# NCAR/SPERR

Hardware: AMD Instinct MI355X
Metric: compress+decompress GB/s/GPU on 256^3 fp32 chunks @ BPP=2.0; bitstream-exact vs ref (higher is better)
Workload: dtype f64; 1 GPU; synthetic 1024^3 fp32 turbulence per GPU, 256^3 chunks, BPP=2.0, step = compress + decompress, volume and container resident in HBM; chunks_per_gpu=64, parallelism=chunks farmed over 1 GPU(s), no collective

## Files before the change

sperr_amd/csrc/engine.hip:

```cpp
#include <algorithm>
#include <array>
#include <chrono>
#include <cstdlib>
#include <cstring>
#include <atomic>
#include <deque>
#include <map>
#include <memory>
#include <condition_variable>
#include <mutex>
#include <numeric>
#include <thread>
#include <string>
#include <vector>

#include "../../include/sperr_hip.h"
#include "engine_internal.h"
#include "host_container.hpp"
#include "speck_dec.h"
#include "dequant.h"
#include "speck_enc.h"
#include "speck_tree_host.hpp"
#include "outlier.h"
#include "quality.h"
// ... 2438 lines not shown
  d.tileStride = round_up(d.nPixTiles, 32);
  TAKE(d.tileLip, uint32_t, d.tileStride * B);
  TAKE(d.tileRef, uint32_t, d.tileStride * B);
  TAKE(d.tileLipOff, uint32_t, d.tileStride * B);
  TAKE(d.tileRefOff, uint32_t, d.tileStride * B);
  {
    uint8_t* tb = nullptr;
    TAKE(tb, uint8_t, d.tileStride * B);
    d.tileBorn = use_tables(P) ? tb : nullptr;
  }
  d.lipResStride = Npad / 64 + 2;
  TAKE(d.lipSig, uint64_t, d.lipResStride * B);
  TAKE(d.lipNeg, uint64_t, d.lipResStride * B);
  d.tokStride = (2 * N + 1 + 63) / 64 + 2;
  TAKE(d.tokMask, uint64_t, d.tokStride * B);
  TAKE(d.tokCnt, uint32_t, d.tokStride * B);
  TAKE(d.tokOff, uint32_t, d.tokStride * B);
  d.tokSegStride = round_up(d.tokStride / 2048 + 2, 32);
  TAKE(d.tokSegSum, uint32_t, d.tokSegStride * B);
  TAKE(d.tokSegBase, uint32_t, d.tokSegStride * B);
  d.streamStride = (size_t)(maxPayloadBytes / 8) + 4;
  TAKE(d.stream, uint64_t, d.streamStride * B);
  d.levelClass = P.d_levelClass;
  d.levelSlot = P.d_levelSlot;
  d.slotLevel = P.d_slotLevel;
  d.nSlots = P.nSlots;
  d.maskWords = (uint32_t)d.streamStride;
  d.maskStride = (size_t)P.nSlots * d.maskWords;
  TAKE(d.mask, uint64_t, std::max<size_t>(d.maskStride, 1) * B);
  d.prefWords = (d.maskWords + 3u) / 4u;
  d.prefStride = (size_t)P.nSlots * d.prefWords;
  TAKE(d.maskPrefix, uint32_t, std::max<size_t>(d.prefStride, 1) * B);
  d.bornStride = P.ht.nsets + 8;
  d.hiGroupsMax = 8;
  d.bornSeg = (uint32_t)((P.ht.nsets + 8) / 16 + 64);
  d.bornPitch = d.bornStride + (size_t)d.bornSeg * d.hiGroupsMax;
  TAKE(d.bornPacked, uint64_t, d.bornPitch * B);
  TAKE(d.bornPosLev, uint64_t, d.bornPitch * B);
  d.lisStamps = nullptr;
  if (g_lis_stamps_on) {
    TAKE(d.lisStamps, uint64_t, 64 * B);
  }
  d.queueCap = 28672 + 64;
  static const int hiKcap = tune_getenv("SPERR_HIP_HI_KCAP") ? std::max(2, atoi(tune_getenv("SPERR_HIP_HI_KCAP"))) : 5;
  d.hiK = (uint32_t)std::min(std::max(2, P.maxK), hiKcap);
  static const uint32_t ahead = tune_getenv("SPERR_HIP_HI_AHEAD") ? (uint32_t)atoi(tune_getenv("SPERR_HIP_HI_AHEAD")) : 512u;
  d.hiAhead = ahead;
  static const uint32_t extra = tune_getenv("SPERR_HIP_HI_EXTRA") ? (uint32_t)atoi(tune_getenv("SPERR_HIP_HI_EXTRA")) : 1u;
  d.hiExtra = extra;
  d.hiHop2 = 0;
  d.hiCand = 1;
  d.hiSmemBytes = 148 * 1024;
  d.hiW = hi_window((int)d.hiK, d.hiSmemBytes, d.hiHop2);
  d.queueStride = (size_t)d.queueCap * 4 * d.hiGroupsMax;
  TAKE(d.queue, uint64_t, d.queueStride * B);
  d.hiAhead = std::min(d.hiAhead / 64 * 64, d.hiW / 2);
  d.hiFlagStride = ((d.streamStride * 64 + N) / std::max<uint32_t>(512u, d.hiW - d.hiAhead) + 12) * 4;
  d.mxSlot = P.d_mxSlot;
  d.mxLevelGroup = P.d_mxLevelGroup;
  d.mxS = kMxS;
  d.mxM = kMxM;
  d.mxQ = kMxQ;
  d.mxSmemBytes = mx_smem_bytes(kMxS, kMxM, kMxQ);
  if (use_mixed(P))
    d.hiFlagStride = std::max<size_t>(d.hiFlagStride, ((d.streamStride * 64 + N) / kMxS + 4) * kMxWordsPerRegion);
  TAKE(d.hiFlags, unsigned long long, d.hiFlagStride * B);
  d.iRoots = P.d_iRoots;
  d.iLevels = P.ht.iLevels;
  d.leafCap = P.ht.nsets + 8;
  d.leafSeg = (uint32_t)((P.ht.nsets + 8) / 16 + 64);
  d.leafStride = d.leafCap + (size_t)d.leafSeg * d.hiGroupsMax;
  TAKE(d.leafEv, uint64_t, d.leafStride * B);
  d.sigbitsStride = P.lisEntries / 64 + 4;
  TAKE(d.sigbits, uint64_t, d.sigbitsStride * B);
  d.l0FlagStride = (d.streamStride * 64 + N) / 4096 + 4;
  TAKE(d.l0Flags, unsigned long long, d.l0FlagStride * B);
  TAKE(d.l0Tab, unsigned long long, d.l0FlagStride * 17 * B);
  d.l0Level = P.l0Level;
  TAKE(d.l1Flags, unsigned long long, d.l0FlagStride * B);
  d.l1Level = P.l1Level;
  TAKE(d.l2Flags, unsigned long long, d.l0FlagStride * B);
  d.l2Level = P.l2Level;
  d.wordLeaf = P.d_wordLeaf;
  d.leafStateStride = round_up(P.ht.nnodes, 64);
  TAKE(d.leafState, uint16_t, d.leafStateStride * B);
  d.leafDirtyStride = d.leafStateStride / 32 + 1;
  TAKE(d.leafDirty, uint8_t, d.leafDirtyStride * B);
#undef TAKE
  return true;
}

int reset_dec_call(const DecBuffers& d, uint32_t nb, hipStream_t ss)
{
  HIP_CHECK(hipMemsetAsync(d.cst, 0, nb * sizeof(CoderState), ss));
  HIP_CHECK(hipMemsetAsync(d.st, 0, nb * sizeof(DecState), ss));
  HIP_CHECK(hipMemsetAsync(d.mask, 0, std::max<size_t>(d.maskStride, 1) * nb * 8, ss));
  HIP_CHECK(hipMemsetAsync(d.l0Flags, 0, d.l0FlagStride * nb * 8, ss));
  HIP_CHECK(hipMemsetAsync(d.l0Tab, 0, d.l0FlagStride * 17 * nb * 8, ss));
  HIP_CHECK(hipMemsetAsync(d.l1Flags, 0, d.l0FlagStride * nb * 8, ss));
  HIP_CHECK(hipMemsetAsync(d.l2Flags, 0, d.l0FlagStride * nb * 8, ss));
  HIP_CHECK(hipMemsetAsync(d.hiFlags, 0, d.hiFlagStride * nb * 8, ss));
  HIP_CHECK(hipMemsetAsync(d.sigbits, 0, d.sigbitsStride * nb * 8, ss));
  if (d.lisStamps)
    HIP_CHECK(hipMemsetAsync(d.lisStamps, 0, 64 * 8 * nb, ss));
  return 0;
}
// ... 2405 lines not shown
```

sperr_amd/csrc/speck_dec.h:

```cpp
#ifndef SPERR_AMD_SPECK_DEC_H
#define SPERR_AMD_SPECK_DEC_H

#include "common.h"

namespace sperrhip {

struct DecState {
  uint32_t active;
  int32_t done;
  uint32_t error;
  int32_t nbp;
  uint32_t cur;
  uint32_t nLip, nRef;
  uint32_t nLeafEv;
  int32_t lastPlane;
  int32_t refPlaneP1;
  uint32_t refPartial;
  uint64_t pos;
  uint64_t avail;
  uint64_t total_bits;
  uint64_t payload;
  uint64_t lipStart, lipBits;
  uint32_t l0Ticket;
  int32_t l0PlaneP1;
// ... 68 lines not shown
  uint32_t* tokOff;
  size_t tokStride;
  uint32_t* tokSegSum;
  uint32_t* tokSegBase;
  size_t tokSegStride;
  const spk::LevelClass* levelClass;
  const uint8_t* levelSlot;
  const uint8_t* slotLevel;
  uint32_t nSlots;
  uint32_t maskWords;
  uint64_t* mask;
  uint32_t* maskPrefix;
  uint32_t prefWords;
  size_t prefStride;
  size_t maskStride;
  uint64_t* bornPacked;
  uint64_t* bornPosLev;
  size_t bornStride;
  size_t bornPitch;
  uint32_t bornSeg;
  uint32_t leafSeg;
  uint64_t* queue;
  uint32_t queueCap;
  size_t queueStride;
  uint64_t* sigbits;
  size_t sigbitsStride;
  uint32_t treeTabLen;
  uint64_t* leafEv;
  uint32_t leafCap;
  size_t leafStride;
  uint16_t* leafState;
  size_t leafStateStride;
  uint8_t* leafDirty;
  size_t leafDirtyStride;
  const uint32_t* wordLeaf;
  unsigned long long* l0Flags;
  size_t l0FlagStride;
  int32_t l0Level;
  unsigned long long* l0Tab;
  unsigned long long* l1Flags;
  int32_t l1Level;
  unsigned long long* l2Flags;
  int32_t l2Level;
  uint64_t* lisStamps;
  unsigned long long* hiFlags;
  size_t hiFlagStride;
  uint32_t hiW;
  uint32_t hiK;
  uint32_t hiSmemBytes;
  uint32_t hiHop2;
  uint32_t hiGroupsMax;
  uint32_t hiExtra;
  uint32_t hiCand;
  uint32_t hiAhead;
  const uint64_t* iRoots;
  uint32_t iLevels;
  const uint8_t* mxSlot;
  const uint8_t* mxLevelGroup;
  uint32_t mxS, mxM;
  uint32_t mxQ;
  uint32_t mxSmemBytes;
};

struct DecPlanHost {
  const uint64_t* d_initLIS;
  const uint32_t* d_initLen;
  bool tables;
  bool l0;
  bool l1;
  int maxK;
  bool hi = false;
  bool l2 = false;
  bool mixed = false;
  uint32_t gridDiv = 1;
  uint32_t mxGroups = 0;
  bool skipFinish = false;
  uint32_t* d_live = nullptr;
  uint32_t* h_live = nullptr;
  hipEvent_t* liveEv = nullptr;
};
constexpr int kLiveSlots = 24;

constexpr int kTabWMax = 28672;
__host__ __device__ inline uint32_t tab_window(int K, uint32_t smemBytes)
{
  const uint32_t perBit8 = 8u * (uint32_t)(2 * (2 * K - 1) + 4) + 1u;
  const uint32_t fixed = 4 * 8 + 130 * 4 + (uint32_t)(2 * K) * 8 + 64;
  uint32_t w = (uint32_t)(((uint64_t)(smemBytes - fixed) * 8) / perBit8);
  w = w / 1024 * 1024;
  if (w > (uint32_t)kTabWMax)
    w = kTabWMax;
  return w;
}

__host__ __device__ inline uint32_t hi_window(int K, uint32_t smemBytes, uint32_t hop2 = 1)
{
  const uint32_t perBit8 = 8u * (uint32_t)(2 * (2 * K - 1) + (hop2 ? 8 : 4)) + 1u;
  const uint32_t fixed = 4 * 8 + 2 * 130 * 4 + (uint32_t)(2 * K) * 8 + 64;
  uint32_t w = (uint32_t)(((uint64_t)(smemBytes - fixed) * 8) / perBit8);
  w = w / 256 * 256;
  if (w > (uint32_t)kTabWMax)
    w = kTabWMax;
  return w;
}

constexpr int kMxWordsPerRegion = 8;
constexpr uint32_t kMxS = 2048, kMxM = 768, kMxQ = 1024, kMxRing = 8192;
uint32_t mx_smem_bytes(uint32_t S, uint32_t M, uint32_t Q);
int prepare_lis_mx(const DecBuffers& b);
int launch_lis_mx(hipStream_t stream, const DecBuffers& b, int p, uint32_t groups, bool stamps);

int launch_speck_decode(hipStream_t stream, const DecBuffers& b, const DecPlanHost& plan,
                        const uint8_t* container, const uint64_t* d_chunkOff,
                        const uint64_t* d_chunkLen, bool wide_pass, int maxPlanes);

}
#endif
```

sperr_amd/csrc/speck_dec.hip:

```cpp
#include "speck_dec.h"
#include "dequant.h"
#include "bit_words.h"
#include "lis_chain.h"

namespace sperrhip {

using namespace spk;

#define DEC_ACTIVE_OR_RETURN(s, p)                               \
  if (!(s).active || (s).done || (int)(p) >= (s).nbp)            \
    return;

__device__ __forceinline__ uint64_t get64(const uint64_t* words, uint64_t pos)
{
  const uint64_t lo = words[pos >> 6];
  const int sh = (int)(pos & 63);
  return sh ? (lo >> sh) | (words[(pos >> 6) + 1] << (64 - sh)) : lo;
}

__global__ void k_dec_header(DecBuffers b, const uint8_t* container, const uint64_t* chunkOff,
                             const uint64_t* chunkLen, const uint64_t* initLIS,
                             const uint32_t* initLen, int wide_pass)
{
  const uint32_t c = blockIdx.x * blockDim.x + threadIdx.x;
// ... 1849 lines not shown
      const LevelClass& B = sh_lc[l];
      const int BK = min((int)B.K, Kcap);
      ok = BK <= tk;
      for (int j = 0; ok && j < BK; j++)
        ok = A.arity[j] == B.arity[j] && A.lev[j] == B.lev[j];
    }
    return __ballot(ok);
  };
  auto tables_serve = [&](int lv) -> bool {
    if (sh_tabLevel < 0)
      return false;
    const LevelClass& A = sh_lc[sh_tabLevel];
    const LevelClass& B = sh_lc[lv];
    const int BK = min((int)B.K, Kcap);
    if (BK > sh_tabK)
      return false;
    for (int j = 0; j < BK; j++)
      if (A.arity[j] != B.arity[j] || A.lev[j] != B.lev[j])
        return false;
    return true;
  };

  const uint32_t segB0 = (uint32_t)b.bornStride + blockIdx.x * b.bornSeg;
  const uint32_t segL0 = b.leafCap + blockIdx.x * b.leafSeg;
  auto born_slots = [&](uint32_t n) -> uint32_t {
    if (n == 0)
      return 0;
    const uint32_t k = atomicAdd(&sh_segBorn, n);
    if (k + n <= b.bornSeg)
      return segB0 + k;
    atomicMin(&sh_segBornEnd, k);
    return atomicAdd(&s.bornCount, n);
  };
  auto leaf_slot = [&]() -> uint32_t {
    const uint32_t k = atomicAdd(&sh_segLeaf, 1u);
    if (k < b.leafSeg)
      return segL0 + k;
    const uint32_t g = atomicAdd(&s.leafCount, 1u);
    return g < b.leafCap ? g : 0xffffffffu;
  };
  auto write_born = [&](uint32_t slot, uint32_t lev, uint64_t abs, uint64_t packed) {
    const uint64_t rel = abs - phase0;
    if (!(slot < b.bornStride || (slot >= segB0 && slot < segB0 + b.bornSeg)))
      return;
    bornPacked[slot] = packed;
    bornPosLev[slot] = ((uint64_t)lev << 48) | rel;
    atomic_or64(b.mask + c * b.maskStride + (size_t)sh_lslot[lev] * b.maskWords + (rel >> 6),
                1ull << (rel & 63));
  };
  auto born_counts = [&](uint32_t lev, uint64_t abs) -> bool {
    return sh_lslot[lev] != 0xff && abs - phase0 < maskBits;
  };

  auto expand_all = [&]() {
    const LevelClass& C = sh_lc[sh_tabLevel];
    for (int round = 0;; round++) {
      const uint32_t nin = sh_qn[round % 3];
      if (nin == 0)
        break;
      if (tid == 0 && b.lisStamps) {
        unsigned long long* o_ = reinterpret_cast<unsigned long long*>(b.lisStamps + (size_t)c * 64);
        atomicAdd(o_ + 44, 1ull);
        atomicAdd(o_ + 45, (unsigned long long)nin);
      }
      const uint64_t* qin = qbuf[round & 1];
      uint64_t* qout = qbuf[(round + 1) & 1];
      for (uint32_t i0 = 0; i0 < nin; i0 += kTabThreads) {
        const uint32_t i = i0 + tid;
        const bool have = i < nin;
        uint64_t ident = 0, meta = 0;
        if (have) {
          ident = qin[i * 2];
          meta = qin[i * 2 + 1];
        }
        const int cls = (int)((meta >> 1) & 0x7f);
        const uint32_t y0 = (uint32_t)(meta >> 8);
        const Node nd = unpack_node(have ? ((meta & 1ull) ? lisCur[ident] : ident) : 0ull);
        const int ar = have ? C.arity[cls] : 0;
        const Grid g = sh_grids[nd.grid];
        const bool isLeaf = have && cls == 0;
        uint32_t sigm = 0, negm = 0;
        if (isLeaf) {
          const uint32_t v = bits.bits32(y0);
          uint32_t yy = 0, found = 0;
          if (ar == 8)
            split8_pixels(v, sigm, negm);
          else {
            for (int k = 0; k < ar; k++) {
              const uint32_t coded = found | (uint32_t)(k + 1 != ar);
              const uint32_t bit = coded ? (v >> yy) & 1u : 1u;
              yy += coded;
              const uint32_t sgn = (v >> yy) & 1u;
              sigm |= bit << k;
              negm |= (bit & (sgn ^ 1u)) << k;
              found |= bit;
              yy += bit;
            }
          }
        }
        const bool isSet = have && cls > 0;
        const uint16_t* Up = Uu + (size_t)(isSet ? cls - 1 : 0) * TS;
        const uint32_t kidLev = isSet ? C.lev[cls - 1] : 0u;
        if (isLeaf) {
          const uint32_t fid = g.nodeOff + ((((uint32_t)nd.i[2] << g.e[1]) + nd.i[1]) << g.e[0]) + nd.i[0];
          const uint32_t slotL = leaf_slot();
          if (slotL != 0xffffffffu)
            leafEv[slotL] = (uint64_t)fid | ((uint64_t)sigm << 32) | ((uint64_t)negm << 40);
        }
        if (isSet) {
          const Root rt = sh_roots[g.root];
          uint32_t cbase[3], cshift[3];
          uint32_t nb = 0;
          for (int ax = 0; ax < 3; ax++) {
            if (g.depth < rt.D[ax]) {
              cbase[ax] = (uint32_t)nd.i[ax] * 2u;
              cshift[ax] = nb++;
            }
            else {
              cbase[ax] = nd.i[ax];
              cshift[ax] = 31;
            }
          }
          const uint64_t gridBits = (uint64_t)(nd.grid + 1) << 48;
          uint32_t y = y0, found = 0;
          for (int k = 0; k < ar; k++) {
            const uint64_t kid = gridBits |
                                 ((uint64_t)(cbase[2] | (((uint32_t)k >> cshift[2]) & 1u)) << 32) |
                                 ((uint64_t)(cbase[1] | (((uint32_t)k >> cshift[1]) & 1u)) << 16) |
                                 (uint64_t)(cbase[0] | (((uint32_t)k >> cshift[0]) & 1u));
            const bool coded = found || (k + 1 != ar);
            uint32_t start = y;
            if (coded) {
              const uint32_t u = Up[y];
              if (!(u & 0x8000u)) {
                if (born_counts(kidLev, a + y))
                  write_born(born_slots(1u), kidLev, a + y, kid);
                y += 1;
                continue;
              }
              start = y + 1;
              y += u & 0x7fffu;
            }
            found = 1;
            const uint32_t slot = atomicAdd(&sh_qn[(round + 1) % 3], 1u);
            if (slot < b.queueCap) {
              qout[slot * 2] = kid;
              qout[slot * 2 + 1] = ((uint64_t)start << 8) | ((uint64_t)(cls - 1) << 1);
            }
          }
        }
      }
      if (tid == 0)
        sh_qn[(round + 2) % 3] = 0;
      __syncthreads();
    }
    if (tid == 0)
      sh_qn[0] = sh_qn[1] = sh_qn[2] = 0;
    __syncthreads();
  };

  const int kSpecExtra = (int)b.hiExtra;
  const bool hiCand = b.hiCand != 0;
  constexpr uint32_t kActDone = 0, kActTables = 1, kActHopTab = 2, kActFlushTables = 4;
  const uint32_t wave = (uint32_t)tid >> 6;

  for (;;) {
    if (tid == 0) {
      const bool over = __hip_atomic_load(&s.hiPlaneP1, __ATOMIC_RELAXED, __HIP_MEMORY_SCOPE_AGENT) == p + 1;
      sh_ticket = over ? kL0None : atomicAdd(&s.hiTicket, 1u);
      sh_any = 0;
      sh_over = 0;
      sh_nlog = 0;
      sh_parInit = 0;
      sh_haveState = 0;
      sh_stop = 0;
      for (int k = 0; k < 8; k++)
        sh_tacc[k] = 0;
      sh_qn[0] = sh_qn[1] = sh_qn[2] = 0;
    }
    __syncthreads();
    const uint32_t i = sh_ticket;
    if (i == kL0None || ((size_t)i + 1) * 4 > b.hiFlagStride)
      break;
    const bool stamps = b.lisStamps != nullptr && tid == 0;
    uint64_t st0 = stamps ? __builtin_readcyclecounter() : 0, st1 = 0;
    {
      uint64_t off = 0;
      uint32_t sz = kHiFirstRegion, j = 0;
      for (; j < i && sz < SRmax; j++, sz <<= 1)
        off += sz;
      if (j < i)
        off += (uint64_t)(i - j) * SRmax;
      SR = min(sz, SRmax);
      if (j < i)
        SR = SRmax;
      W = SR + b.hiAhead;
      a = S0 + off;
    }
    bits.q0 = (uint32_t)(a & 63);
    {
      const uint64_t w0 = a >> 6;
      uint64_t any = 0;
// ... 1405 lines not shown
```

sperr_amd/csrc/speck_enc.hip:

```cpp
#include "speck_enc.h"

namespace sperrhip {

using namespace spk;

#define ACTIVE_OR_RETURN(s, p)                                     \
  if (!(s).active || (s).done || (int)(p) >= (s).nbp)              \
    return;

__global__ void k_enc_state_init(EncBuffers b, const uint64_t* initLIS, const uint32_t* initLen,
                                 uint64_t budget, int wide_pass)
{
  const uint32_t c = blockIdx.x * blockDim.x + threadIdx.x;
  if (c >= b.nchunks)
    return;
  EncState& s = b.st[c];
  const CoderState& cs = b.cst[c];
  s.active = wide_pass ? (cs.need_retry != 0) : (cs.is_const == 0 && cs.need_retry == 0);
  s.nbp = 0;
  s.done = 0;
  s.plast = 0;
  s.bornCount = 0;
  s.pos = 0;
  s.total_bits = 0;
  s.budget = budget;
  s.lisBits = 0;
  s.cur = 0;
  s.iPart = b.iLevels;
  for (int q = 0; q < kMaxPlanes; q++)
    s.bucketCnt[q] = 0;
  for (uint32_t l = 0; l < b.tree.nlevels; l++) {
    s.listLen[0][l] = initLen[l];
    s.listLen[1][l] = 0;
    s.bornTot[l] = 0;
    for (uint32_t k = 0; k < initLen[l]; k++)
      b.lis[0][c * b.lisStride + b.levelOff[l] + k] = initLIS[b.levelOff[l] + k];
  }
}

struct OctKids {
  int m[8];
  uint32_t e[8];
  uint32_t base, sy, sz;
  bool deepest;
};

__device__ __forceinline__ uint32_t oct_kid(const OctKids& k, int j)
{
  return k.base + (uint32_t)(j & 1) + (uint32_t)((j >> 1) & 1) * k.sy + (uint32_t)(j >> 2) * k.sz;
}

__device__ __forceinline__ void oct_load(const Tree& t, const Grid& g, const Root& r, const Node& nd,
                                         const int8_t* M, const uint32_t* E, const int8_t* msb,
// ... 364 lines not shown
            v = (pc & 0xffffffffull) | ((uint64_t)((uint32_t)(pc >> 32) + b.koff[c * b.nodeStride + id]) << 32);
          }
        }
        chain[id] = v;
      }
    }
    ids[q] = id;
    bins[q] = mine ? m : -1;
    ranks[q] = wave_hist_add(h, bins[q]);
  }
  __syncthreads();
  if (threadIdx.x < kMaxPlanes && h[threadIdx.x])
    base[threadIdx.x] = atomicAdd(&s.bucketCur[threadIdx.x], h[threadIdx.x]);
  __syncthreads();
#pragma unroll
  for (int q = 0; q < kNodePerMax; q++)
    if (bins[q] >= 0)
      b.bucket[c * b.nodeStride + base[bins[q]] + ranks[q]] = ids[q];
}

__global__ void k_enc_planes_setup(EncBuffers b)
{
  const uint32_t c = blockIdx.x * blockDim.x + threadIdx.x;
  if (c >= b.nchunks)
    return;
  EncState& s = b.st[c];
  if (!s.active)
    return;
  const Tree& t = b.tree;
  int nbp = 0;
  for (uint32_t r = 0; r < t.nroots; r++)
    nbp = max(nbp, (int)b.M[c * b.nodeStride + t.grids[t.roots[r].gridFirst].nodeOff] + 1);
  s.nbp = nbp;
  s.plast = nbp;
  if (nbp == 0) {
    s.done = 1;
    s.total_bits = 0;
  }
}

__device__ __forceinline__ void load_pix(const int8_t* a, uint32_t i0, uint32_t n, int v[kPixPer])
{
  static_assert(kPixPer == 16, "one 16-byte load per thread");
  if (i0 + kPixPer <= n) {
    const uint4 q = *reinterpret_cast<const uint4*>(a + i0);
    const uint32_t w[4] = {q.x, q.y, q.z, q.w};
#pragma unroll
    for (int k = 0; k < kPixPer; k++)
      v[k] = (int)(int8_t)(w[k >> 2] >> ((k & 3) * 8));
  }
  else
    for (int k = 0; k < kPixPer; k++)
      v[k] = (i0 + k < n) ? a[i0 + k] : -1;
}

__global__ void __launch_bounds__(kThreads) k_census(EncBuffers b, int maxPlanes)
{
  const uint32_t c = blockIdx.y;
  const EncState& s = b.st[c];
  if (!s.active)
    return;
  __shared__ uint32_t hist[kThreads / 64][2][kMaxPlanes + 1];
  for (uint32_t i = threadIdx.x; i < (kThreads / 64) * 2 * (kMaxPlanes + 1); i += kThreads)
    (&hist[0][0][0])[i] = 0;
  __syncthreads();
  const uint32_t n = b.tree.nvals;
  const uint32_t i0 = blockIdx.x * kPixTile + threadIdx.x * kPixPer;
  const int wave = threadIdx.x >> 6;
  uint32_t zeroM = 0, zeroB = 0;
  if (i0 < n) {
    int m[kPixPer], bp[kPixPer];
    load_pix(b.msb + c * b.pixStride, i0, n, m);
    load_pix(b.bplane + c * b.pixStride, i0, n, bp);
#pragma unroll
    for (int k = 0; k < kPixPer; k++)
      if (i0 + k < n) {
        if (m[k] < 0)
          zeroM++;
        else
          atomicAdd(&hist[wave][0][m[k] + 1], bp[k] > m[k] ? 0x10001u : 1u);
      }
#pragma unroll
    for (int k = 0; k < kPixPer; k += 2) {
      const bool a = i0 + k < n, c2 = i0 + k + 1 < n;
      if (a && c2 && bp[k] == bp[k + 1]) {
        if (bp[k] < 0)
          zeroB += 2;
        else
          atomicAdd(&hist[wave][1][bp[k] + 1], 2u);
      }
      else {
        if (a) {
          if (bp[k] < 0)
            zeroB++;
          else
            atomicAdd(&hist[wave][1][bp[k] + 1], 1u);
        }
        if (c2) {
          if (bp[k + 1] < 0)
            zeroB++;
          else
            atomicAdd(&hist[wave][1][bp[k + 1] + 1], 1u);
        }
      }
    }
  }
// ... 780 lines not shown

__global__ void __launch_bounds__(kThreads) k_mask_scan(EncBuffers b, int p)
{
  const uint32_t c = blockIdx.y, slot = blockIdx.x;
  EncState& s = b.st[c];
  ACTIVE_OR_RETURN(s, p);
  __shared__ uint32_t sm[kThreads / 64 + 1];
  const uint64_t nbits = min(s.lisBits, (uint64_t)b.maskWords * 64);
  const uint32_t nwords = (uint32_t)((nbits + 63) / 64);
  const uint64_t* mask = b.mask + c * b.maskStride + (size_t)slot * b.maskWords;
  uint32_t* pre = b.maskPrefix + c * b.prefStride + (size_t)slot * b.prefWords;
  uint32_t carry = 0;
  for (uint32_t base = 0; base < nwords; base += kThreads * 4) {
    uint32_t v[4], tsum = 0;
    for (int k = 0; k < 4; k++) {
      const uint32_t i = base + threadIdx.x * 4 + k;
      v[k] = i < nwords ? (uint32_t)__popcll(mask[i]) : 0u;
      tsum += v[k];
    }
    uint32_t total;
    const uint32_t ex = block_exclusive_scan<uint32_t>(tsum, sm, &total) + carry;
    if (base + threadIdx.x * 4 < nwords)
      pre[base / 4 + threadIdx.x] = ex;
    carry += total;
  }
  if (threadIdx.x == 0)
    s.bornTot[b.slotLevel[slot]] = carry;
}

__global__ void __launch_bounds__(kThreads) k_born_place(EncBuffers b, int p)
{
  const uint32_t c = blockIdx.y;
  const EncState& s = b.st[c];
  ACTIVE_OR_RETURN(s, p);
  const uint32_t nx = s.cur ^ 1u;
  for (uint32_t k = blockIdx.x * blockDim.x + threadIdx.x; k < s.bornCount;
       k += gridDim.x * blockDim.x) {
    const uint64_t pl = b.bornPosLev[c * b.bornStride + k];
    const uint32_t lev = (uint32_t)(pl >> 48);
    const uint64_t rel = pl & ((1ull << 48) - 1);
    const uint32_t slot = b.levelSlot[lev];
    const uint32_t wi = (uint32_t)(rel >> 6);
    const size_t mo = c * b.maskStride + (size_t)slot * b.maskWords + wi;
    uint32_t rank = b.maskPrefix[c * b.prefStride + (size_t)slot * b.prefWords + (wi >> 2)] +
                    (uint32_t)__popcll(b.mask[mo] & ((1ull << (rel & 63)) - 1ull));
    for (uint32_t j = 1; j <= (wi & 3u); j++)
      rank += (uint32_t)__popcll(b.mask[mo - j]);
    b.lis[nx][c * b.lisStride + b.levelOff[lev] + s.listLen[nx][lev] + rank] =
        b.bornPacked[c * b.bornStride + k];
  }
}


template <typename CT>
__global__ void __launch_bounds__(kThreads) k_emit_pixels(EncBuffers b)
{
  const uint32_t c = blockIdx.y;
  const EncState& s = b.st[c];
  if (!s.active || s.nbp == 0)
    return;
  constexpr int kWords = kPixTile * 2 / 64 + 2;
  __shared__ unsigned long long lipw[kWords], refw[kWords];
  __shared__ uint32_t sm[kThreads / 64 + 1];
  const uint32_t n = b.tree.nvals;
  const uint32_t tile = blockIdx.x;
  const uint32_t i0 = tile * kPixTile + threadIdx.x * kPixPer;
  int m[kPixPer], bp[kPixPer];
  load_pix(b.bplane + c * b.pixStride, i0, n, bp);
  int bpmax = -1;
#pragma unroll
  for (int k = 0; k < kPixPer; k++)
    bpmax = max(bpmax, bp[k]);
  const bool live = bpmax > s.plast;
  CT cf[kPixPer];
  uint32_t sg = 0;
  const CT* coef = reinterpret_cast<const CT*>(b.coef) + c * b.coefStride;
  const uint64_t* sign = b.sign + c * b.signStride;
#pragma unroll
  for (int k = 0; k < kPixPer; k++) {
    m[k] = -1;
    cf[k] = (CT)0;
  }
  if (live) {
    load_pix(b.msb + c * b.pixStride, i0, n, m);
    if (i0 < n)
      sg = (uint32_t)(sign[i0 >> 6] >> (i0 & 63));
#pragma unroll
    for (int k = 0; k < kPixPer; k++)
      cf[k] = (i0 + k < n) ? coef[i0 + k] : (CT)0;
  }
  else
    bpmax = -1;
  uint32_t M[7], B[7];
#pragma unroll
  for (int j = 0; j < 7; j++) {
    M[j] = B[j] = 0;
#pragma unroll
    for (int k = 0; k < kPixPer; k++) {
      M[j] |= (((uint32_t)(m[k] + 1) >> j) & 1u) << k;
      B[j] |= (((uint32_t)(bp[k] + 1) >> j) & 1u) << k;
    }
  }
  auto above_equal = [](const uint32_t (&X)[7], uint32_t t, uint32_t& gt, uint32_t& eq) {
    gt = 0;
    eq = 0xffffu;
#pragma unroll
    for (int j = 6; j >= 0; j--) {
      if ((t >> j) & 1u)
        eq &= X[j];
      else {
        gt |= eq & X[j];
        eq &= ~X[j];
      }
    }
  };
  __shared__ uint8_t pextLut[16][16];
  {
    const uint32_t mk = threadIdx.x >> 4, vl = threadIdx.x & 15u;
    uint32_t r = 0, o = 0;
    for (int i = 0; i < 4; i++)
      if ((mk >> i) & 1u) {
        r |= ((vl >> i) & 1u) << o;
        o++;
      }
    pextLut[mk][vl] = (uint8_t)r;
  }
  static_assert(kThreads == 256, "one pext table entry per thread");
  auto pext16 = [&](uint32_t val, uint32_t mask) -> uint32_t {
    uint32_t r = 0, sh = 0;
#pragma unroll
    for (int i = 0; i < 4; i++) {
      const uint32_t mn = (mask >> (4 * i)) & 15u;
      r |= (uint32_t)pextLut[mn][(val >> (4 * i)) & 15u] << sh;
      sh += (uint32_t)__popc(mn);
    }
    return r;
  };
  auto plane_bits = [&](int pl, bool withRef, uint32_t& lbits, uint32_t& lval, uint32_t& rbits, uint32_t& rval) {
    uint32_t gtM, eqM, gtB, eqB;
    above_equal(M, (uint32_t)pl + 1u, gtM, eqM);
    above_equal(B, (uint32_t)pl + 1u, gtB, eqB);
    const uint32_t inLip = gtB & ~gtM;
    lbits = lval = rbits = rval = 0;
    if (inLip) {
      const uint32_t nl = (uint32_t)__popc(inLip);
      uint32_t tok = pext16(eqM, inLip);
      uint32_t sgn = pext16(sg, inLip);
      lbits = nl;
      lval = tok;
      for (uint32_t rest = tok; rest;) {
        const uint32_t i = 31u - (uint32_t)__clz((int)rest);
        rest &= ~(1u << i);
        const uint32_t low = lval & ((2u << i) - 1u);
        lval = low | (((sgn >> i) & 1u) << (i + 1)) | ((lval >> (i + 1)) << (i + 2));
        lbits++;
      }
    }
    if (withRef && gtM) {
      uint32_t cbit = 0;
#pragma unroll
      for (int k = 0; k < kPixPer; k++)
        cbit |= (uint32_t)((cf[k] >> pl) & 1) << k;
      rbits = (uint32_t)__popc(gtM);
      rval = pext16(cbit, gtM);
    }
  };
  const uint32_t* cnt = b.pixCnt + c * b.pixCntStride;
  const uint32_t* off = b.pixOff + c * b.pixCntStride;
  uint64_t* stream = b.stream + c * b.streamStride;
  __shared__ uint32_t tcnt[2 * kMaxPlanes];
  __shared__ uint64_t tbase[2 * kMaxPlanes];
  const int nbp = s.nbp, plast = s.plast;
  for (int t = threadIdx.x; t < 2 * nbp; t += blockDim.x) {
    const int pp = t >> 1;
    const bool ref = (t & 1) != 0;
    tcnt[t] = (ref && !s.rec[pp].didREF) ? 0u : cnt[(size_t)t * b.nPixTiles + tile];
    tbase[t] = (ref ? s.rec[pp].baseREF : s.rec[pp].baseLIP) + off[(size_t)t * b.nPixTiles + tile];
  }
  const uint64_t budget = s.budget;
  const uint64_t limitWord = (budget >> 6) + ((budget & 63) ? 1 : 0);
  __shared__ unsigned long long lipw2[kWords], refw2[kWords];
  for (int w = threadIdx.x; w < kWords; w += blockDim.x)
    lipw[w] = refw[w] = lipw2[w] = refw2[w] = 0;
  __shared__ uint64_t sm64[kThreads / 64 + 1];
  __syncthreads();
  for (int p = nbp - 1; p >= plast; p -= 2) {
    const int q = p - 1;
    const bool two = q >= plast;
    const uint32_t nlipA = tcnt[p * 2], nrefA = tcnt[p * 2 + 1];
    const uint32_t nlipB = two ? tcnt[q * 2] : 0u, nrefB = two ? tcnt[q * 2 + 1] : 0u;
    if ((nlipA | nrefA | nlipB | nrefB) == 0)
      continue;
    uint32_t lbA = 0, lvA = 0, rbA = 0, rvA = 0, lbB = 0, lvB = 0, rbB = 0, rvB = 0;
    if (q < bpmax) {
      plane_bits(p, nrefA != 0, lbA, lvA, rbA, rvA);
      if (two)
        plane_bits(q, nrefB != 0, lbB, lvB, rbB, rvB);
    }
    if (!nrefA)
      rbA = 0;
    if (!nrefB)
      rbB = 0;
    uint64_t total;
    const uint64_t ex = block_exclusive_scan_lds<uint64_t>((uint64_t)lbA | ((uint64_t)rbA << 16) | ((uint64_t)lbB << 32) |
                                                           ((uint64_t)rbB << 48), sm64, &total);
    const uint64_t lipBaseA = tbase[p * 2], refBaseA = tbase[p * 2 + 1];
    const uint64_t lipBaseB = two ? tbase[q * 2] : 0ull, refBaseB = two ? tbase[q * 2 + 1] : 0ull;
    auto deposit = [&](unsigned long long* w, uint32_t val, uint32_t nbits, uint32_t at) {
      atomicOr(&w[at >> 6], (unsigned long long)val << (at & 63));
      if ((at & 63) + nbits > 64)
        atomicOr(&w[(at >> 6) + 1], (unsigned long long)val >> (64 - (at & 63)));
    };
    if (lvA)
      deposit(lipw, lvA, lbA, (uint32_t)(ex & 0xffffu) + (uint32_t)(lipBaseA & 63));
    if (rvA && nrefA)
      deposit(refw, rvA, rbA, (uint32_t)((ex >> 16) & 0xffffu) + (uint32_t)(refBaseA & 63));
    if (lvB)
      deposit(lipw2, lvB, lbB, (uint32_t)((ex >> 32) & 0xffffu) + (uint32_t)(lipBaseB & 63));
    if (rvB && nrefB)
      deposit(refw2, rvB, rbB, (uint32_t)(ex >> 48) + (uint32_t)(refBaseB & 63));
    LDS_ONLY_BARRIER();
    auto flush = [&](unsigned long long* w, uint64_t base, uint32_t n) {
      if (n == 0)
        return;
      const uint64_t firstW = base >> 6, lastW = (base + n - 1) >> 6;
      for (int i = threadIdx.x; i < kWords; i += blockDim.x) {
        uint64_t v = w[i];
        if (v == 0)
          continue;
        w[i] = 0;
        const uint64_t gw = firstW + i;
        if (gw < limitWord) {
          if (gw == limitWord - 1 && (budget & 63))
            v &= (1ull << (budget & 63)) - 1;
          if (gw == firstW || gw >= lastW)
            atomic_or64(stream + gw, v);
          else
            stream[gw] = v;
        }
      }
    };
    flush(lipw, lipBaseA, nlipA);
    flush(refw, refBaseA, nrefA);
    if (two) {
      flush(lipw2, lipBaseB, nlipB);
      flush(refw2, refBaseB, nrefB);
    }
    LDS_ONLY_BARRIER();
  }
}


__global__ void k_enc_finalize(EncBuffers b, uint64_t raw_budget, int rate_mode, int wide_pass)
{
  const uint32_t c = blockIdx.x * blockDim.x + threadIdx.x;
  if (c >= b.nchunks)
    return;
  EncState& s = b.st[c];
  CoderState& cs = b.cst[c];
  if (cs.is_const) {
    cs.stream_len = 17;
    cs.need_retry = 0;
    return;
  }
  if (!s.active)
    return;
  const uint64_t keep = min(s.total_bits, s.budget);
  const uint64_t payload = (keep + 7) / 8;
  cs.stream_len = 17 + 9 + payload;
  cs.nbp = s.nbp;
  cs.total_bits = s.total_bits;
  if (rate_mode)
    cs.need_retry = (!wide_pass && (9 + payload) * 8 < raw_budget) ? 1u : 0u;
}

__global__ void __launch_bounds__(kThreads) k_enc_bound(EncBuffers b, uint32_t* out)
{
  __shared__ uint32_t lo, hi;
  if (threadIdx.x == 0) {
    lo = 0xffffffffu;
    hi = 0;
  }
  __syncthreads();
  for (uint32_t c = threadIdx.x; c < b.nchunks; c += blockDim.x) {
    const EncState& s = b.st[c];
    if (!s.active || s.nbp <= 0)
      continue;
    int p = s.nbp - 1;
    uint64_t cum = 0;
    for (; p > 0; p--) {
      cum += s.lipTot[p] + s.refTot[p];
      if (cum >= s.budget)
        break;
    }
    atomicMin(&lo, (uint32_t)p);
    atomicMax(&hi, (uint32_t)s.nbp);
  }
  __syncthreads();
  if (threadIdx.x == 0) {
    out[0] = lo == 0xffffffffu ? 0u : lo;
    out[1] = hi;
// ... 161 lines not shown
```

Before: 67.57 GB/s.

## Split expand_all into leaf and set passes, spill queue into LDS hop buffer

Restructures the decoder's hi-level tree expansion so leaf nodes and set nodes are handled in separate passes. Set nodes are expanded with eight threads per node, one child each, instead of one thread walking all children serially. Child queue entries now go first into an LDS ring carved from the hop buffer, sized by a new cap and overridable by environment variable, and overflow to the global queue. This aims to cut per-thread serial loops and global-memory queue traffic. It adds redundant per-sub-thread prefix scans and risks correctness if the hop buffer is in use during expansion.

```diff
diff --git a/sperr_amd/csrc/engine.hip b/sperr_amd/csrc/engine.hip
--- a/sperr_amd/csrc/engine.hip
+++ b/sperr_amd/csrc/engine.hip
@@ -2514,6 +2514,10 @@
   d.hiCand = 1;
   d.hiSmemBytes = 148 * 1024;
   d.hiW = hi_window((int)d.hiK, d.hiSmemBytes, d.hiHop2);
+  static const int ldsq = getenv("SPERR_HIP_HI_LDSQ") ? std::max(0, atoi(getenv("SPERR_HIP_HI_LDSQ"))) : -1;
+  d.hiLdsq = hi_ldsq_cap(d.hiW, d.hiHop2);
+  if (ldsq >= 0)
+    d.hiLdsq = std::min(d.hiLdsq, (uint32_t)ldsq);
   d.queueStride = (size_t)d.queueCap * 4 * d.hiGroupsMax;
   TAKE(d.queue, uint64_t, d.queueStride * B);
   d.hiAhead = std::min(d.hiAhead / 64 * 64, d.hiW / 2);
diff --git a/sperr_amd/csrc/speck_dec.h b/sperr_amd/csrc/speck_dec.h
--- a/sperr_amd/csrc/speck_dec.h
+++ b/sperr_amd/csrc/speck_dec.h
@@ -144,6 +144,7 @@
   uint32_t hiGroupsMax;
   uint32_t hiExtra;
   uint32_t hiCand;
+  uint32_t hiLdsq;
   uint32_t hiAhead;
   const uint64_t* iRoots;
   uint32_t iLevels;
@@ -195,6 +196,10 @@
     w = kTabWMax;
   return w;
 }
+__host__ __device__ inline uint32_t hi_ldsq_cap(uint32_t W, uint32_t hop2)
+{
+  return (hop2 ? 2u : 1u) * (W + 130u) * 4u / 32u;
+}
 
 constexpr int kMxWordsPerRegion = 8;
 constexpr uint32_t kMxS = 2048, kMxM = 768, kMxQ = 1024, kMxRing = 8192;
diff --git a/sperr_amd/csrc/speck_dec.hip b/sperr_amd/csrc/speck_dec.hip
--- a/sperr_amd/csrc/speck_dec.hip
+++ b/sperr_amd/csrc/speck_dec.hip
@@ -1925,102 +1925,127 @@
     return sh_lslot[lev] != 0xff && abs - phase0 < maskBits;
   };
 
+  const uint32_t ldsq = min(b.hiLdsq, hi_ldsq_cap(Wmax, b.hiHop2));
+  uint64_t* const lq = reinterpret_cast<uint64_t*>(hop);
   auto expand_all = [&]() {
     const LevelClass& C = sh_lc[sh_tabLevel];
+    if (ldsq != 0 && tid == 0)
+      sh_hopTop[0] = sh_hopTop[1] = -1;
     for (int round = 0;; round++) {
-      const uint32_t nin = sh_qn[round % 3];
+      const uint32_t nlds = round == 0 ? 0u : ldsq;
+      const uint32_t nin = min(sh_qn[round % 3], nlds + b.queueCap);
       if (nin == 0)
         break;
       if (tid == 0 && b.lisStamps) {
         unsigned long long* o_ = reinterpret_cast<unsigned long long*>(b.lisStamps + (size_t)c * 64);
         atomicAdd(o_ + 44, 1ull);
         atomicAdd(o_ + 45, (unsigned long long)nin);
+        atomicAdd(o_ + 46, (unsigned long long)min(nin, nlds));
+        atomicAdd(o_ + 47, (unsigned long long)(round == 0 ? 0u : nin - min(nin, nlds)));
       }
       const uint64_t* qin = qbuf[round & 1];
       uint64_t* qout = qbuf[(round + 1) & 1];
+      const uint32_t lin = (uint32_t)(round & 1) * 2u * ldsq;
+      const uint32_t lout = (uint32_t)((round + 1) & 1) * 2u * ldsq;
+      auto item = [&](uint32_t i, uint64_t& ident, uint64_t& meta) {
+        if (i < nlds) {
+          ident = lq[lin + i];
+          meta = lq[lin + ldsq + i];
+        }
+        else {
+          ident = qin[(i - nlds) * 2];
+          meta = qin[(i - nlds) * 2 + 1];
+        }
+      };
       for (uint32_t i0 = 0; i0 < nin; i0 += kTabThreads) {
         const uint32_t i = i0 + tid;
-        const bool have = i < nin;
+        uint64_t ident = 0, meta = 2;
+        if (i < nin)
+          item(i, ident, meta);
+        const int cls = (int)((meta >> 1) & 0x7f);
+        if (cls != 0)
+          continue;
+        const Node nd = unpack_node((meta & 1ull) ? lisCur[ident] : ident);
+        const int ar = C.arity[0];
+        const Grid g = sh_grids[nd.grid];
+        const uint32_t v = bits.bits32((uint32_t)(meta >> 8));
+        uint32_t sigm = 0, negm = 0;
+        if (ar == 8)
+          split8_pixels(v, sigm, negm);
+        else {
+          uint32_t yy = 0, found = 0;
+          for (int k = 0; k < ar; k++) {
+            const uint32_t coded = found | (uint32_t)(k + 1 != ar);
+            const uint32_t bit = coded ? (v >> yy) & 1u : 1u;
+            yy += coded;
+            const uint32_t sgn = (v >> yy) & 1u;
+            sigm |= bit << k;
+            negm |= (bit & (sgn ^ 1u)) << k;
+            found |= bit;
+            yy += bit;
+          }
+        }
+        const uint32_t fid = g.nodeOff + ((((uint32_t)nd.i[2] << g.e[1]) + nd.i[1]) << g.e[0]) + nd.i[0];
+        const uint32_t slotL = leaf_slot();
+        if (slotL != 0xffffffffu)
+          leafEv[slotL] = (uint64_t)fid | ((uint64_t)sigm << 32) | ((uint64_t)negm << 40);
+      }
+      for (uint32_t i0 = 0; i0 < nin; i0 += kTabThreads / 8) {
+        const uint32_t i = i0 + ((uint32_t)tid >> 3), sub = (uint32_t)tid & 7u;
         uint64_t ident = 0, meta = 0;
-        if (have) {
-          ident = qin[i * 2];
-          meta = qin[i * 2 + 1];
-        }
+        if (i < nin)
+          item(i, ident, meta);
         const int cls = (int)((meta >> 1) & 0x7f);
-        const uint32_t y0 = (uint32_t)(meta >> 8);
-        const Node nd = unpack_node(have ? ((meta & 1ull) ? lisCur[ident] : ident) : 0ull);
-        const int ar = have ? C.arity[cls] : 0;
+        if (cls == 0)
+          continue;
+        const Node nd = unpack_node((meta & 1ull) ? lisCur[ident] : ident);
+        const uint32_t ar = C.arity[cls];
+        const uint16_t* Up = Uu + (size_t)(cls - 1) * TS;
+        uint32_t y = (uint32_t)(meta >> 8), found = 0, at = 0;
+        bool born = false;
+        for (uint32_t k = 0; k < ar; k++) {
+          uint32_t len = 0, kAt = y;
+          bool kBorn = false;
+          if (found || k + 1 != ar) {
+            const uint32_t u = Up[y];
+            kBorn = !(u & 0x8000u);
+            len = kBorn ? 1u : (u & 0x7fffu);
+            kAt = kBorn ? y : y + 1;
+          }
+          found |= (uint32_t)!kBorn;
+          if (k == sub) {
+            at = kAt;
+            born = kBorn;
+          }
+          y += len;
+        }
+        if (sub >= ar)
+          continue;
         const Grid g = sh_grids[nd.grid];
-        const bool isLeaf = have && cls == 0;
-        uint32_t sigm = 0, negm = 0;
-        if (isLeaf) {
-          const uint32_t v = bits.bits32(y0);
-          uint32_t yy = 0, found = 0;
-          if (ar == 8)
-            split8_pixels(v, sigm, negm);
-          else {
-            for (int k = 0; k < ar; k++) {
-              const uint32_t coded = found | (uint32_t)(k + 1 != ar);
-              const uint32_t bit = coded ? (v >> yy) & 1u : 1u;
-              yy += coded;
-              const uint32_t sgn = (v >> yy) & 1u;
-              sigm |= bit << k;
-              negm |= (bit & (sgn ^ 1u)) << k;
-              found |= bit;
-              yy += bit;
-            }
-          }
-        }
-        const bool isSet = have && cls > 0;
-        const uint16_t* Up = Uu + (size_t)(isSet ? cls - 1 : 0) * TS;
-        const uint32_t kidLev = isSet ? C.lev[cls - 1] : 0u;
-        if (isLeaf) {
-          const uint32_t fid = g.nodeOff + ((((uint32_t)nd.i[2] << g.e[1]) + nd.i[1]) << g.e[0]) + nd.i[0];
-          const uint32_t slotL = leaf_slot();
-          if (slotL != 0xffffffffu)
-            leafEv[slotL] = (uint64_t)fid | ((uint64_t)sigm << 32) | ((uint64_t)negm << 40);
-        }
-        if (isSet) {
-          const Root rt = sh_roots[g.root];
-          uint32_t cbase[3], cshift[3];
-          uint32_t nb = 0;
-          for (int ax = 0; ax < 3; ax++) {
-            if (g.depth < rt.D[ax]) {
-              cbase[ax] = (uint32_t)nd.i[ax] * 2u;
-              cshift[ax] = nb++;
-            }
-            else {
-              cbase[ax] = nd.i[ax];
-              cshift[ax] = 31;
-            }
-          }
-          const uint64_t gridBits = (uint64_t)(nd.grid + 1) << 48;
-          uint32_t y = y0, found = 0;
-          for (int k = 0; k < ar; k++) {
-            const uint64_t kid = gridBits |
-                                 ((uint64_t)(cbase[2] | (((uint32_t)k >> cshift[2]) & 1u)) << 32) |
-                                 ((uint64_t)(cbase[1] | (((uint32_t)k >> cshift[1]) & 1u)) << 16) |
-                                 (uint64_t)(cbase[0] | (((uint32_t)k >> cshift[0]) & 1u));
-            const bool coded = found || (k + 1 != ar);
-            uint32_t start = y;
-            if (coded) {
-              const uint32_t u = Up[y];
-              if (!(u & 0x8000u)) {
-                if (born_counts(kidLev, a + y))
-                  write_born(born_slots(1u), kidLev, a + y, kid);
-                y += 1;
-                continue;
-              }
-              start = y + 1;
-              y += u & 0x7fffu;
-            }
-            found = 1;
-            const uint32_t slot = atomicAdd(&sh_qn[(round + 1) % 3], 1u);
-            if (slot < b.queueCap) {
-              qout[slot * 2] = kid;
-              qout[slot * 2 + 1] = ((uint64_t)start << 8) | ((uint64_t)(cls - 1) << 1);
-            }
-          }
+        const Root rt = sh_roots[g.root];
+        uint32_t ci[3], nb = 0;
+        for (int ax = 0; ax < 3; ax++) {
+          if (g.depth < rt.D[ax])
+            ci[ax] = (uint32_t)nd.i[ax] * 2u | ((sub >> nb++) & 1u);
+          else
+            ci[ax] = nd.i[ax];
+        }
+        const uint64_t kid = ((uint64_t)(nd.grid + 1) << 48) | ((uint64_t)ci[2] << 32) | ((uint64_t)ci[1] << 16) | (uint64_t)ci[0];
+        if (born) {
+          const uint32_t kidLev = C.lev[cls - 1];
+          if (born_counts(kidLev, a + at))
+            write_born(born_slots(1u), kidLev, a + at, kid);
+          continue;
+        }
+        const uint32_t slot = atomicAdd(&sh_qn[(round + 1) % 3], 1u);
+        const uint64_t kmeta = ((uint64_t)at << 8) | ((uint64_t)(cls - 1) << 1);
+        if (slot < ldsq) {
+          lq[lout + slot] = kid;
+          lq[lout + ldsq + slot] = kmeta;
+        }
+        else if (slot - ldsq < b.queueCap) {
+          qout[(slot - ldsq) * 2] = kid;
+          qout[(slot - ldsq) * 2 + 1] = kmeta;
         }
       }
       if (tid == 0)
```

Result: no change. 67.51 GB/s (-0.1%).

## Bit-transpose coefficients into planes and table-drive sign interleave in pixel emit

Applied to the files above, without the earlier changes.

For 32-bit coefficients, the pixel emit kernel now loads 16 coefficients with vector loads and bit-transposes them into 16-bit plane masks. Significance (gt/eq) is then tracked incrementally per plane instead of loading the msb array and recomputing comparisons, and the birth-plane masks are built with packed SWAR arithmetic. The serial per-bit sign-insertion loop is replaced by a 256-entry LDS lookup table, and per-plane counts and bases are made wave-uniform with readfirstlane. An occupancy hint is added, along with EMIT_PIX_OFF debug macros that are off by default; these add register pressure and extra code paths.

```diff
diff --git a/sperr_amd/csrc/pix_planes.h b/sperr_amd/csrc/pix_planes.h
--- /dev/null
+++ b/sperr_amd/csrc/pix_planes.h
@@ -0,0 +1,93 @@
+#ifndef SPERR_AMD_PIX_PLANES_H
+#define SPERR_AMD_PIX_PLANES_H
+
+#include <stdint.h>
+
+#if defined(__HIPCC__)
+#define PP_HD __host__ __device__ __forceinline__
+#else
+#define PP_HD inline
+#endif
+
+namespace sperrhip {
+
+PP_HD void pix_transpose16(uint32_t (&r)[16])
+{
+#define PP_SWAP_STAGE(S, MASK)                                   \
+  _Pragma("unroll") for (int i = 0; i < 16; i++) if (!(i & S)) { \
+    const uint32_t t = ((r[i] >> S) ^ r[i + S]) & MASK;          \
+    r[i + S] ^= t;                                               \
+    r[i] ^= t << S;                                              \
+  }
+  PP_SWAP_STAGE(8, 0x00ff00ffu)
+  PP_SWAP_STAGE(4, 0x0f0f0f0fu)
+  PP_SWAP_STAGE(2, 0x33333333u)
+  PP_SWAP_STAGE(1, 0x55555555u)
+#undef PP_SWAP_STAGE
+}
+
+PP_HD uint32_t pix_plane(const uint32_t (&P)[16], int pl)
+{
+  return (P[pl & 15] >> (pl & 16)) & 0xffffu;
+}
+
+PP_HD void pix_msb_step(uint32_t cp, uint32_t& gt, uint32_t& eq)
+{
+  eq = cp & ~gt;
+  gt |= cp;
+}
+
+PP_HD uint8_t pix_pext_entry(uint32_t mk, uint32_t vl)
+{
+  uint32_t r = 0, o = 0;
+  for (int i = 0; i < 4; i++)
+    if ((mk >> i) & 1u) {
+      r |= ((vl >> i) & 1u) << o;
+      o++;
+    }
+  return (uint8_t)r;
+}
+
+template <typename LUT>
+PP_HD uint32_t pix_pext16(const LUT& lut, uint32_t val, uint32_t mask)
+{
+  uint32_t r = 0, sh = 0;
+#pragma unroll
+  for (int i = 0; i < 4; i++) {
+    const uint32_t mn = (mask >> (4 * i)) & 15u;
+    r |= (uint32_t)lut[mn * 16 + ((val >> (4 * i)) & 15u)] << sh;
+    sh += (uint32_t)__builtin_popcount(mn);
+  }
+  return r;
+}
+
+PP_HD uint8_t pix_sign_entry(uint32_t tn, uint32_t sn)
+{
+  uint32_t r = 0, o = 0;
+  for (int i = 0; i < 4; i++) {
+    r |= ((tn >> i) & 1u) << o;
+    o++;
+    if ((tn >> i) & 1u) {
+      r |= ((sn >> i) & 1u) << o;
+      o++;
+    }
+  }
+  return (uint8_t)r;
+}
+
+template <typename LUT>
+PP_HD uint32_t pix_sign_expand(const LUT& lut, uint32_t tok, uint32_t sgn)
+{
+  uint32_t r = 0, sh = 0;
+#pragma unroll
+  for (int i = 0; i < 4; i++) {
+    const uint32_t tn = (tok >> (4 * i)) & 15u;
+    r |= (uint32_t)lut[tn * 16 + ((sgn >> (4 * i)) & 15u)] << sh;
+    sh += 4u + (uint32_t)__builtin_popcount(tn);
+  }
+  return r;
+}
+
+}
+
+#endif
diff --git a/sperr_amd/csrc/speck_enc.hip b/sperr_amd/csrc/speck_enc.hip
--- a/sperr_amd/csrc/speck_enc.hip
+++ b/sperr_amd/csrc/speck_enc.hip
@@ -1,4 +1,5 @@
 #include "speck_enc.h"
+#include "pix_planes.h"
 
 namespace sperrhip {
 
@@ -469,6 +470,23 @@
   else
     for (int k = 0; k < kPixPer; k++)
       v[k] = (i0 + k < n) ? a[i0 + k] : -1;
+}
+
+__device__ __forceinline__ void load_pix_packed(const int8_t* a, uint32_t i0, uint32_t n, uint32_t (&w)[4])
+{
+  static_assert(kPixPer == 16, "one 16-byte load per thread");
+  if (i0 + kPixPer <= n) {
+    const uint4 q = *reinterpret_cast<const uint4*>(a + i0);
+    w[0] = q.x;
+    w[1] = q.y;
+    w[2] = q.z;
+    w[3] = q.w;
+  }
+  else {
+    w[0] = w[1] = w[2] = w[3] = 0;
+    for (int k = 0; k < kPixPer; k++)
+      w[k >> 2] |= (uint32_t)((i0 + k < n) ? (uint8_t)a[i0 + k] : 0xffu) << ((k & 3) * 8);
+  }
 }
 
 __global__ void __launch_bounds__(kThreads) k_census(EncBuffers b, int maxPlanes)
@@ -1355,60 +1373,119 @@
 }
 
 
+#ifndef EMIT_PIX_OFF
+#define EMIT_PIX_OFF 0
+#endif
 template <typename CT>
-__global__ void __launch_bounds__(kThreads) k_emit_pixels(EncBuffers b)
-{
+__global__ void __launch_bounds__(kThreads) __attribute__((amdgpu_waves_per_eu(sizeof(CT) == 4 ? 7 : 4, 8)))
+k_emit_pixels(EncBuffers b)
+{
+  constexpr bool kPlanes = sizeof(CT) == 4;
   const uint32_t c = blockIdx.y;
   const EncState& s = b.st[c];
   if (!s.active || s.nbp == 0)
     return;
   constexpr int kWords = kPixTile * 2 / 64 + 2;
   __shared__ unsigned long long lipw[kWords], refw[kWords];
-  __shared__ uint32_t sm[kThreads / 64 + 1];
   const uint32_t n = b.tree.nvals;
   const uint32_t tile = blockIdx.x;
   const uint32_t i0 = tile * kPixTile + threadIdx.x * kPixPer;
-  int m[kPixPer], bp[kPixPer];
-  load_pix(b.bplane + c * b.pixStride, i0, n, bp);
+  constexpr int kBirthBits = kPlanes ? 6 : 7;
+  uint32_t B[kBirthBits];
   int bpmax = -1;
-#pragma unroll
-  for (int k = 0; k < kPixPer; k++)
-    bpmax = max(bpmax, bp[k]);
+  {
+    uint32_t w[4];
+    load_pix_packed(b.bplane + c * b.pixStride, i0, n, w);
+#pragma unroll
+    for (int k = 0; k < kPixPer; k++)
+      bpmax = max(bpmax, (int)(int8_t)(w[k >> 2] >> ((k & 3) * 8)));
+#pragma unroll
+    for (int i = 0; i < 4; i++)
+      w[i] = ((w[i] & 0x7f7f7f7fu) + 0x01010101u) & 0x7f7f7f7fu;
+#pragma unroll
+    for (int j = 0; j < kBirthBits; j++) {
+      B[j] = 0;
+#pragma unroll
+      for (int i = 0; i < 4; i++)
+        B[j] |= ((((w[i] >> j) & 0x01010101u) * 0x01020408u) >> 24 & 15u) << (4 * i);
+    }
+  }
   const bool live = bpmax > s.plast;
-  CT cf[kPixPer];
   uint32_t sg = 0;
   const CT* coef = reinterpret_cast<const CT*>(b.coef) + c * b.coefStride;
   const uint64_t* sign = b.sign + c * b.signStride;
-#pragma unroll
-  for (int k = 0; k < kPixPer; k++) {
-    m[k] = -1;
-    cf[k] = (CT)0;
-  }
-  if (live) {
-    load_pix(b.msb + c * b.pixStride, i0, n, m);
-    if (i0 < n)
-      sg = (uint32_t)(sign[i0 >> 6] >> (i0 & 63));
-#pragma unroll
-    for (int k = 0; k < kPixPer; k++)
-      cf[k] = (i0 + k < n) ? coef[i0 + k] : (CT)0;
-  }
-  else
-    bpmax = -1;
-  uint32_t M[7], B[7];
-#pragma unroll
-  for (int j = 0; j < 7; j++) {
-    M[j] = B[j] = 0;
+  uint32_t P[kPlanes ? 16 : 1];
+  CT cf[kPlanes ? 1 : kPixPer];
+  uint32_t M[kPlanes ? 1 : 7];
+  if constexpr (kPlanes) {
+#pragma unroll
+    for (int k = 0; k < 16; k++)
+      P[k] = 0;
+    if (live) {
+#if EMIT_PIX_OFF & 1
+#pragma unroll
+      for (int k = 0; k < kPixPer; k++) {
+        const uint32_t h = (i0 + k) * 2654435761u, top = (B[0] >> k & 1u) | (B[1] >> k & 1u) << 1 | (B[2] >> k & 1u) << 2 |
+                                                         (B[3] >> k & 1u) << 3 | (B[4] >> k & 1u) << 4 | (B[5] >> k & 1u) << 5;
+        P[k] = top ? (h >> 7) & (0xffffffffu >> (32u - min(top, 32u))) : 0u;
+      }
+      sg = i0 * 40503u;
+#else
+      if (i0 < n)
+        sg = (uint32_t)(sign[i0 >> 6] >> (i0 & 63));
+      if (i0 + kPixPer <= n) {
+#pragma unroll
+        for (int k = 0; k < kPixPer; k += 4) {
+          const uint4 q = *reinterpret_cast<const uint4*>(coef + i0 + k);
+          P[k] = q.x;
+          P[k + 1] = q.y;
+          P[k + 2] = q.z;
+          P[k + 3] = q.w;
+        }
+      }
+      else {
+#pragma unroll
+        for (int k = 0; k < kPixPer; k++)
+          P[k] = (i0 + k < n) ? coef[i0 + k] : 0u;
+      }
+#endif
+      pix_transpose16(P);
+    }
+    else
+      bpmax = -1;
+  }
+  else {
+    int m[kPixPer];
 #pragma unroll
     for (int k = 0; k < kPixPer; k++) {
-      M[j] |= (((uint32_t)(m[k] + 1) >> j) & 1u) << k;
-      B[j] |= (((uint32_t)(bp[k] + 1) >> j) & 1u) << k;
-    }
-  }
-  auto above_equal = [](const uint32_t (&X)[7], uint32_t t, uint32_t& gt, uint32_t& eq) {
+      m[k] = -1;
+      cf[k] = (CT)0;
+    }
+    if (live) {
+      if (i0 < n)
+        sg = (uint32_t)(sign[i0 >> 6] >> (i0 & 63));
+#pragma unroll
+      for (int k = 0; k < kPixPer; k++) {
+        cf[k] = (i0 + k < n) ? coef[i0 + k] : (CT)0;
+        m[k] = cf[k] ? 63 - __clzll((long long)cf[k]) : -1;
+      }
+    }
+    else
+      bpmax = -1;
+#pragma unroll
+    for (int j = 0; j < 7; j++) {
+      M[j] = 0;
+#pragma unroll
+      for (int k = 0; k < kPixPer; k++)
+        M[j] |= (((uint32_t)(m[k] + 1) >> j) & 1u) << k;
+    }
+  }
+  auto above_equal = [](const auto& X, uint32_t t, uint32_t& gt, uint32_t& eq) {
+    constexpr int NB = (int)(sizeof(X) / sizeof(X[0]));
     gt = 0;
     eq = 0xffffu;
 #pragma unroll
-    for (int j = 6; j >= 0; j--) {
+    for (int j = NB - 1; j >= 0; j--) {
       if ((t >> j) & 1u)
         eq &= X[j];
       else {
@@ -1417,55 +1494,25 @@
       }
     }
   };
-  __shared__ uint8_t pextLut[16][16];
-  {
-    const uint32_t mk = threadIdx.x >> 4, vl = threadIdx.x & 15u;
-    uint32_t r = 0, o = 0;
-    for (int i = 0; i < 4; i++)
-      if ((mk >> i) & 1u) {
-        r |= ((vl >> i) & 1u) << o;
-        o++;
-      }
-    pextLut[mk][vl] = (uint8_t)r;
-  }
-  static_assert(kThreads == 256, "one pext table entry per thread");
-  auto pext16 = [&](uint32_t val, uint32_t mask) -> uint32_t {
-    uint32_t r = 0, sh = 0;
-#pragma unroll
-    for (int i = 0; i < 4; i++) {
-      const uint32_t mn = (mask >> (4 * i)) & 15u;
-      r |= (uint32_t)pextLut[mn][(val >> (4 * i)) & 15u] << sh;
-      sh += (uint32_t)__popc(mn);
-    }
-    return r;
-  };
-  auto plane_bits = [&](int pl, bool withRef, uint32_t& lbits, uint32_t& lval, uint32_t& rbits, uint32_t& rval) {
-    uint32_t gtM, eqM, gtB, eqB;
-    above_equal(M, (uint32_t)pl + 1u, gtM, eqM);
+  __shared__ uint8_t pextLut[256], signLut[256];
+  pextLut[threadIdx.x] = pix_pext_entry(threadIdx.x >> 4, threadIdx.x & 15u);
+  signLut[threadIdx.x] = pix_sign_entry(threadIdx.x >> 4, threadIdx.x & 15u);
+  static_assert(kThreads == 256, "one table entry per thread");
+  auto plane_bits = [&](int pl, uint32_t gtM, uint32_t eqM, uint32_t cbit, bool withRef, uint32_t& lbits, uint32_t& lval,
+                        uint32_t& rbits, uint32_t& rval) {
+    uint32_t gtB, eqB;
     above_equal(B, (uint32_t)pl + 1u, gtB, eqB);
     const uint32_t inLip = gtB & ~gtM;
     lbits = lval = rbits = rval = 0;
     if (inLip) {
-      const uint32_t nl = (uint32_t)__popc(inLip);
-      uint32_t tok = pext16(eqM, inLip);
-      uint32_t sgn = pext16(sg, inLip);
-      lbits = nl;
-      lval = tok;
-      for (uint32_t rest = tok; rest;) {
-        const uint32_t i = 31u - (uint32_t)__clz((int)rest);
-        rest &= ~(1u << i);
-        const uint32_t low = lval & ((2u << i) - 1u);
-        lval = low | (((sgn >> i) & 1u) << (i + 1)) | ((lval >> (i + 1)) << (i + 2));
-        lbits++;
-      }
+      const uint32_t tok = pix_pext16(pextLut, eqM, inLip);
+      lbits = (uint32_t)__popc(inLip) + (uint32_t)__popc(tok);
+      if (tok)
+        lval = pix_sign_expand(signLut, tok, pix_pext16(pextLut, sg, inLip));
     }
     if (withRef && gtM) {
-      uint32_t cbit = 0;
-#pragma unroll
-      for (int k = 0; k < kPixPer; k++)
-        cbit |= (uint32_t)((cf[k] >> pl) & 1) << k;
       rbits = (uint32_t)__popc(gtM);
-      rval = pext16(cbit, gtM);
+      rval = pix_pext16(pextLut, cbit, gtM);
     }
   };
   const uint32_t* cnt = b.pixCnt + c * b.pixCntStride;
@@ -1487,28 +1534,69 @@
     lipw[w] = refw[w] = lipw2[w] = refw2[w] = 0;
   __shared__ uint64_t sm64[kThreads / 64 + 1];
   __syncthreads();
+  auto uni32 = [](uint32_t v) { return (uint32_t)__builtin_amdgcn_readfirstlane((int)v); };
+  auto uni64 = [&](uint64_t v) { return (uint64_t)uni32((uint32_t)v) | ((uint64_t)uni32((uint32_t)(v >> 32)) << 32); };
+  uint32_t gt = 0;
   for (int p = nbp - 1; p >= plast; p -= 2) {
     const int q = p - 1;
     const bool two = q >= plast;
-    const uint32_t nlipA = tcnt[p * 2], nrefA = tcnt[p * 2 + 1];
-    const uint32_t nlipB = two ? tcnt[q * 2] : 0u, nrefB = two ? tcnt[q * 2 + 1] : 0u;
+    uint32_t gtA = 0, eqA = 0, cA = 0, gtB2 = 0, eqB2 = 0, cB = 0;
+    if constexpr (kPlanes) {
+      cA = pix_plane(P, p);
+      cB = pix_plane(P, q);
+      gtA = gt;
+      pix_msb_step(cA, gt, eqA);
+      gtB2 = gt;
+      pix_msb_step(cB, gt, eqB2);
+    }
+    const uint32_t nlipA = uni32(tcnt[p * 2]), nrefA = uni32(tcnt[p * 2 + 1]);
+    const uint32_t nlipB = two ? uni32(tcnt[q * 2]) : 0u, nrefB = two ? uni32(tcnt[q * 2 + 1]) : 0u;
     if ((nlipA | nrefA | nlipB | nrefB) == 0)
       continue;
     uint32_t lbA = 0, lvA = 0, rbA = 0, rvA = 0, lbB = 0, lvB = 0, rbB = 0, rvB = 0;
+#if !(EMIT_PIX_OFF & 2)
     if (q < bpmax) {
-      plane_bits(p, nrefA != 0, lbA, lvA, rbA, rvA);
-      if (two)
-        plane_bits(q, nrefB != 0, lbB, lvB, rbB, rvB);
-    }
+#pragma unroll
+      for (int j = 0; j < kBirthBits; j++)
+        asm volatile("" : "+v"(B[j]));
+      asm volatile("" : "+v"(sg));
+      if constexpr (!kPlanes) {
+        above_equal(M, (uint32_t)p + 1u, gtA, eqA);
+        if (nrefA && gtA) {
+#pragma unroll
+          for (int k = 0; k < kPixPer; k++)
+            cA |= (uint32_t)((cf[k] >> p) & 1) << k;
+        }
+      }
+      plane_bits(p, gtA, eqA, cA, nrefA != 0, lbA, lvA, rbA, rvA);
+      if (two) {
+        if constexpr (!kPlanes) {
+          above_equal(M, (uint32_t)q + 1u, gtB2, eqB2);
+          if (nrefB && gtB2) {
+#pragma unroll
+            for (int k = 0; k < kPixPer; k++)
+              cB |= (uint32_t)((cf[k] >> q) & 1) << k;
+          }
+        }
+        plane_bits(q, gtB2, eqB2, cB, nrefB != 0, lbB, lvB, rbB, rvB);
+      }
+    }
+#endif
     if (!nrefA)
       rbA = 0;
     if (!nrefB)
       rbB = 0;
     uint64_t total;
+#if EMIT_PIX_OFF & 4
+    const uint64_t ex = (uint64_t)threadIdx.x * 0x0010002000100020ull;
+    total = 0;
+#else
     const uint64_t ex = block_exclusive_scan_lds<uint64_t>((uint64_t)lbA | ((uint64_t)rbA << 16) | ((uint64_t)lbB << 32) |
                                                            ((uint64_t)rbB << 48), sm64, &total);
-    const uint64_t lipBaseA = tbase[p * 2], refBaseA = tbase[p * 2 + 1];
-    const uint64_t lipBaseB = two ? tbase[q * 2] : 0ull, refBaseB = two ? tbase[q * 2 + 1] : 0ull;
+#endif
+    const uint64_t lipBaseA = uni64(tbase[p * 2]), refBaseA = uni64(tbase[p * 2 + 1]);
+    const uint64_t lipBaseB = two ? uni64(tbase[q * 2]) : 0ull, refBaseB = two ? uni64(tbase[q * 2 + 1]) : 0ull;
+#if !(EMIT_PIX_OFF & 8)
     auto deposit = [&](unsigned long long* w, uint32_t val, uint32_t nbits, uint32_t at) {
       atomicOr(&w[at >> 6], (unsigned long long)val << (at & 63));
       if ((at & 63) + nbits > 64)
@@ -1550,6 +1638,10 @@
       flush(refw2, refBaseB, nrefB);
     }
     LDS_ONLY_BARRIER();
+#else
+    if (total == 0x123456789ull + lipBaseA + refBaseA + lipBaseB + refBaseB + ex + lvA + rvA + lvB + rvB)
+      stream[0] = ex;
+#endif
   }
 }
 
```

Measured after the change: 67.25 GB/s before, 68.88 GB/s after, median of 6. +2.4%, better.
